# guptakhil/show-tell

Hardware: AMD Instinct MI355X
Metric: training images/sec (ResNet101+GRU, emb=512, bs=128) at 1/2/4/8 MI355X (higher is better)
Workload: dtype bf16; 1 GPU; BASELINE configs[1]: ResNet-101 (train-mode BN, frozen) + 5-layer GRU decoder, E=H=512, V=10000, fwd+bwd+SGD step, synthetic COCO-shaped batch; batch_per_gpu=128, global_batch=128, image=3x224x224, parallelism=dp1

## Files before the change

show-tell_amd/csrc/conv_img.hip:

```cpp
#include "common.h"
#include "prof.h"
#include <stdlib.h>
#include <stdio.h>

namespace {

struct ImgArgs {
  const bf16_t* x; const bf16_t* w; bf16_t* y;
  float* stats; int srep;
  const float* scale; const float* shift; int relu;
  const float* in_stats; const float* in_gamma; const float* in_beta; float in_count, in_eps; int in_srep;
  int B, H, W, N, Wp, R, bands, nbn;
  unsigned long long* stamps;
};

template <int CTRL> __device__ __forceinline__ float dpp_rot_(float v) {
  return __int_as_float(__builtin_amdgcn_update_dpp(0, __float_as_int(v), CTRL, 0xf, 0xf, true));
}
__device__ __forceinline__ float row16_sum_(float v) {
  v += dpp_rot_<0x128>(v); v += dpp_rot_<0x124>(v); v += dpp_rot_<0x122>(v); v += dpp_rot_<0x121>(v);
  return v;
}
__device__ __forceinline__ f32x4 mfma_bf16(const u32x4& a, const u32x4& b, const f32x4& c) {
  return __builtin_amdgcn_mfma_f32_16x16x32_bf16(*reinterpret_cast<const bf16x8*>(&a), *reinterpret_cast<const bf16x8*>(&b), c, 0, 0, 0);
}

template <int NC, int BNLOC>
__device__ __forceinline__ void block_stats_flush(const float (&es)[NC], const float (&ess)[NC], bool writer, int local, char* smem,
                                                  float* sdst, int chan0, int N, int tid) {
  float* sred = reinterpret_cast<float*>(smem);
  __syncthreads();
  if (writer) {
#pragma unroll
    for (int c = 0; c < NC; ++c) { sred[local + c] = es[c]; sred[BNLOC + local + c] = ess[c]; }
  }
  __syncthreads();
  for (int t = tid; t < 2 * BNLOC; t += 256) atomicAdd(sdst + (t < BNLOC ? chan0 + t : N + chan0 + t - BNLOC), sred[t]);
}

__device__ __forceinline__ void bn_relu_chunk(u32x4& v, const float* sc, const float* sh);

template <int C, int TM, int NTW, int HALVES, bool AFFINE, int MS = 1>
__device__ __forceinline__ void conv3x3_img_body(const ImgArgs& a) {
  constexpr int TMW = TM / MS;
  static_assert(TM % MS == 0 && (MS == 1 || MS == 2) && (MS == 1 || HALVES == 1), "position split");
  constexpr int PIX = 2 * C + 32;
  constexpr int CS = C / 32;
  constexpr int CSH = CS / HALVES;
  constexpr int KS = 9 * CS;
  constexpr int CH8 = C / 8;
  constexpr int PSTEP = 256 / CH8;
  constexpr bool ALLW = KS * NTW * 4 <= 96;
  extern __shared__ __attribute__((aligned(16))) char smem[];

  const int tid = threadIdx.x, lane = tid & 63;
  const int wid = __builtin_amdgcn_readfirstlane(tid >> 6);
  int lid;
  {
    const int nblk = gridDim.x, id = blockIdx.x, xcd = id & 7, q = nblk >> 3, r = nblk & 7;
    lid = (xcd < r ? xcd * (q + 1) : r * (q + 1) + (xcd - r) * q) + (id >> 3);
  }
  const int nb = lid % a.nbn;
  const int bi = lid / a.nbn;
  const int band = bi % a.bands, img = bi / a.bands;
  const int r0 = band * a.R;
  const int rows = a.H - r0 < a.R ? a.H - r0 : a.R;
  const int Wp = a.Wp;

#define IMG_STAMP(i) do { if (a.stamps && lane == 0) a.stamps[((size_t)blockIdx.x * 4 + wid) * 8 + (i)] = __builtin_amdgcn_s_memtime(); } while (0)
  IMG_STAMP(0);
  constexpr int NSH = C > 256 ? C / 256 : 1;
  StatHead shd[NSH];
  if (a.in_stats) {
#pragma unroll
    for (int k = 0; k < NSH; ++k) { const int c = (tid + 256 * k) % C; stat_head_issue(shd[k], a.in_stats, a.in_srep, C, c, a.in_gamma, a.in_beta); }
  }
  const int r16 = lane & 15, q4 = lane >> 4;
  const int wn = MS == 1 ? wid : (wid & 1), wm = MS == 1 ? 0 : (wid >> 1);
  const int T0 = (nb * (4 / MS) + wn) * NTW;
  const u32x4* wl = reinterpret_cast<const u32x4*>(a.w) + lane;
  constexpr int WQ = ALLW ? KS : CS;
  u32x4 wq[WQ][NTW];
#pragma unroll
  for (int s = 0; s < WQ; ++s)
#pragma unroll
    for (int j = 0; j < NTW; ++j) wq[s][j] = wl[((size_t)(T0 + j) * KS + s) * 64];

  constexpr int CHH = CH8 / 2, U2 = TM >= 14 ? 19 : TM + 3;
  u32x4 v1[HALVES == 2 ? U2 : 1]; bool ok1[HALVES == 2 ? U2 : 1];
  float sc1[8], sh1[8];
  const int cch2 = tid % CHH, pp2 = tid / CHH;
  const bool xf_ = a.in_stats != nullptr;
  if constexpr (HALVES == 2) {
    const int total = 16 * TM + 2 * Wp + 2;
    float* coef = reinterpret_cast<float*>(smem + (size_t)total * PIX);
    const bf16_t* ximg = a.x + (size_t)img * a.H * a.W * C + cch2 * 8;
    u32x4 v0[U2];
    int pr = pp2 / Wp, pc = pp2 - pr * Wp;
#pragma unroll
    for (int u = 0; u < U2; ++u) {
      const int hi = r0 - 1 + pr, wi = pc - 1;
      ok1[u] = pr < rows + 2 && (unsigned)hi < (unsigned)a.H && (unsigned)wi < (unsigned)a.W;
      const int hc = hi < 0 ? 0 : (hi >= a.H ? a.H - 1 : hi), wc = wi < 0 ? 0 : (wi >= a.W ? a.W - 1 : wi);
      v0[u] = *reinterpret_cast<const u32x4*>(ximg + (size_t)(hc * a.W + wc) * C);
      v1[u] = *reinterpret_cast<const u32x4*>(ximg + (size_t)(hc * a.W + wc) * C + C / 2);
      if (!ok1[u]) { v0[u] = u32x4{0u, 0u, 0u, 0u}; v1[u] = u32x4{0u, 0u, 0u, 0u}; }
      pc += 16;
      while (pc >= Wp) { pc -= Wp; ++pr; }
    }
    float sc0[8], sh0[8];
    if (xf_) {
      const float inv = 1.0f / a.in_count;
#pragma unroll
      for (int k = 0; k < NSH; ++k) {
        const int c = tid + 256 * k;
        if (c < C) stat_head_finish(shd[k], a.in_stats, a.in_srep, C, c, inv, a.in_eps, coef[c], coef[C + c]);
      }
      __syncthreads();
#pragma unroll
      for (int e = 0; e < 8; ++e) {
        sc0[e] = coef[cch2 * 8 + e]; sh0[e] = coef[C + cch2 * 8 + e];
        sc1[e] = coef[C / 2 + cch2 * 8 + e]; sh1[e] = coef[C + C / 2 + cch2 * 8 + e];
      }
    }
#pragma unroll
    for (int u = 0; u < U2; ++u) {
      if (xf_ && ok1[u]) bn_relu_chunk(v0[u], sc0, sh0);
      if (pp2 + 16 * u < total) *reinterpret_cast<u32x4*>(smem + (size_t)(pp2 + 16 * u) * PIX + cch2 * 16) = v0[u];
    }
  } else
  {
    const int cch = tid % CH8;
    float sc[8], sh[8];
    const bool xf = a.in_stats != nullptr;
    const int total = 16 * TM + 2 * Wp + 2;
    float* coef = reinterpret_cast<float*>(smem + (size_t)total * PIX);
    const bf16_t* ximg = a.x + (size_t)img * a.H * a.W * C + cch * 8;
    int pp = tid / CH8;
    int pr = pp / Wp, pc = pp - pr * Wp;
    constexpr int U = C == 256 ? 33 : C == 128 ? 18 : C == 64 ? 12 : 21;
    bool first = true;
    for (; pp < total; pp += U * PSTEP) {
      u32x4 v[U]; bool ok[U]; int dst[U];
#pragma unroll
      for (int u = 0; u < U; ++u) {
        const int hi = r0 - 1 + pr, wi = pc - 1;
        ok[u] = pr < rows + 2 && (unsigned)hi < (unsigned)a.H && (unsigned)wi < (unsigned)a.W;
        dst[u] = pp + u * PSTEP < total ? (pp + u * PSTEP) * PIX + cch * 16 : -1;
        const int hc = hi < 0 ? 0 : (hi >= a.H ? a.H - 1 : hi), wc = wi < 0 ? 0 : (wi >= a.W ? a.W - 1 : wi);
        v[u] = *reinterpret_cast<const u32x4*>(ximg + (size_t)(hc * a.W + wc) * C);
        if (!ok[u]) v[u] = u32x4{0u, 0u, 0u, 0u};
        pc += PSTEP;
        while (pc >= Wp) { pc -= Wp; ++pr; }
      }
      if (xf && first) {
        const float inv = 1.0f / a.in_count;
#pragma unroll
        for (int k = 0; k < NSH; ++k) {
          const int c = tid + 256 * k;
          if (c < C) stat_head_finish(shd[k], a.in_stats, a.in_srep, C, c, inv, a.in_eps, coef[c], coef[C + c]);
        }
        __syncthreads();
#pragma unroll
        for (int e = 0; e < 8; ++e) { sc[e] = coef[cch * 8 + e]; sh[e] = coef[C + cch * 8 + e]; }
        first = false;
      }
#pragma unroll
      for (int u = 0; u < U; ++u) {
        if (xf && ok[u]) {
#pragma unroll
          for (int d = 0; d < 4; ++d) {
            const float lo = fmaxf(__uint_as_float(v[u][d] << 16) * sc[2 * d] + sh[2 * d], 0.f);
            const float hi = fmaxf(__uint_as_float(v[u][d] & 0xffff0000u) * sc[2 * d + 1] + sh[2 * d + 1], 0.f);
            v[u][d] = pack_bf16x2(lo, hi);
          }
        }
        if (dst[u] >= 0) *reinterpret_cast<u32x4*>(smem + dst[u]) = v[u];
      }
    }
  }
  IMG_STAMP(1);
  __syncthreads();
  IMG_STAMP(2);

  f32x4 acc[TMW][NTW];
#pragma unroll
  for (int i = 0; i < TMW; ++i)
#pragma unroll
    for (int j = 0; j < NTW; ++j) acc[i][j] = f32x4{0.f, 0.f, 0.f, 0.f};

  constexpr int TH = TMW > 7 ? 7 : TMW;
  const char* abase = smem + (wm * TMW * 16 + r16) * PIX + q4 * 16;
  auto read_a = [&](u32x4 (&fa)[TMW], int s) {
    const int half = s / (9 * CSH), tap = (s / CSH) % 9, cs = half * CSH + s % CSH;
    const char* ab = abase + ((tap / 3) * Wp + tap % 3) * PIX;
    const char* ab2 = ab + TH * 16 * PIX;
#pragma unroll
    for (int i = 0; i < TMW; ++i)
      fa[i] = i < TH ? *reinterpret_cast<const u32x4*>(ab + i * 16 * PIX + cs * 64) : *reinterpret_cast<const u32x4*>(ab2 + (i - TH) * 16 * PIX + cs * 64);
  };
  u32x4 fa0[TMW], fa1[TMW];
  read_a(fa0, 0);
#pragma clang loop unroll(full)
  for (int s = 0; s < KS; ++s) {
    u32x4 (&cur)[TMW] = (s & 1) ? fa1 : fa0;
    u32x4 (&nxt)[TMW] = (s & 1) ? fa0 : fa1;
    constexpr int SPLIT = HALVES == 2 ? KS / 2 : -1;
    if (s + 1 < KS && s + 1 != SPLIT) read_a(nxt, s + 1);
#pragma unroll
    for (int i = 0; i < TMW; ++i)
#pragma unroll
      for (int j = 0; j < NTW; ++j) acc[i][j] = mfma_bf16(wq[s % WQ][j], cur[i], acc[i][j]);
    if (s + WQ < KS) {
#pragma unroll
      for (int j = 0; j < NTW; ++j) wq[s % WQ][j] = wl[((size_t)(T0 + j) * KS + s + WQ) * 64];
    }
    if constexpr (HALVES == 2) {
      if (s < U2) {
        if (xf_ && ok1[s]) bn_relu_chunk(v1[s], sc1, sh1);
        if (pp2 + 16 * s < 16 * TM + 2 * Wp + 2) *reinterpret_cast<u32x4*>(smem + (size_t)(pp2 + 16 * s) * PIX + C + cch2 * 16) = v1[s];
      }
    }
    __builtin_amdgcn_sched_barrier(0);
    if constexpr (HALVES == 2) {
      if (s + 1 == SPLIT) { __syncthreads(); read_a(nxt, s + 1); }
    }
  }

  IMG_STAMP(3);
  constexpr int NC = 4 * NTW;
  const int cb = T0 * 16 + NC * q4;
  float es[NC], ess[NC], scv[NC], shv[NC];
#pragma unroll
  for (int c = 0; c < NC; ++c) { es[c] = 0.f; ess[c] = 0.f; scv[c] = 1.f; shv[c] = 0.f; }
  if constexpr (AFFINE) {
#pragma unroll
    for (int c = 0; c < NC; ++c) { scv[c] = a.scale[cb + c]; shv[c] = a.shift[cb + c]; }
#pragma unroll
    for (int c = 0; c < NC; ++c) asm volatile("" : "+v"(scv[c]), "+v"(shv[c]));
  }
  int ho = r0, wo = r16 + wm * TMW * 16;
  while (wo >= Wp) { wo -= Wp; ++ho; }
  const long yimg = ((long)img * a.H * a.W * a.N + cb) * 2;
#pragma unroll
  for (int i = 0; i < TMW; ++i) {
    const bool valid = wo < a.W && ho < r0 + rows;
    if (valid) {
      float v[NC];
#pragma unroll
      for (int j = 0; j < NTW; ++j)
#pragma unroll
        for (int e = 0; e < 4; ++e) v[4 * j + e] = acc[i][j][e];
#pragma unroll
      for (int c = 0; c < NC; ++c) { es[c] += v[c]; ess[c] += v[c] * v[c]; }
      if constexpr (AFFINE) {
#pragma unroll
        for (int c = 0; c < NC; ++c) v[c] = v[c] * scv[c] + shv[c];
        if (a.relu) {
#pragma unroll
          for (int c = 0; c < NC; ++c) v[c] = fmaxf(v[c], 0.f);
        }
      }
      const long dst = yimg + (long)(ho * a.W + wo) * a.N * 2;
      if constexpr (NTW == 1) {
        st_out_store8(a.y, dst, u32x2{pack_bf16x2(v[0], v[1]), pack_bf16x2(v[2], v[3])});
      } else {
#pragma unroll
        for (int h = 0; h < NTW / 2; ++h)
          st_out_store16(a.y, dst + 16 * h, u32x4{pack_bf16x2(v[8 * h], v[8 * h + 1]), pack_bf16x2(v[8 * h + 2], v[8 * h + 3]),
                                                  pack_bf16x2(v[8 * h + 4], v[8 * h + 5]), pack_bf16x2(v[8 * h + 6], v[8 * h + 7])});
      }
    }
    wo += 16;
    while (wo >= Wp) { wo -= Wp; ++ho; }
  }
  if (a.stats) {
    float* sdst = a.stats + (a.srep > 1 ? (size_t)(bi % a.srep) * 2 * a.N : 0);
#pragma unroll
    for (int c = 0; c < NC; ++c) { es[c] = row16_sum_(es[c]); ess[c] = row16_sum_(ess[c]); }
    if constexpr (MS == 1) {
      block_stats_flush<NC, 64 * NTW>(es, ess, r16 == 0, wid * 16 * NTW + NC * q4, smem, sdst, nb * 64 * NTW, a.N, tid);
    } else {
      constexpr int BNLOC = (4 / MS) * 16 * NTW;
      float* sred = reinterpret_cast<float*>(smem);
      const int local = wn * 16 * NTW + NC * q4;
      __syncthreads();
      if (r16 == 0 && wm == 0) {
#pragma unroll
        for (int c = 0; c < NC; ++c) { sred[local + c] = es[c]; sred[BNLOC + local + c] = ess[c]; }
      }
      __syncthreads();
      if (r16 == 0 && wm == 1) {
#pragma unroll
        for (int c = 0; c < NC; ++c) { sred[local + c] += es[c]; sred[BNLOC + local + c] += ess[c]; }
      }
      __syncthreads();
      const int chan0 = nb * BNLOC;
      for (int t = tid; t < 2 * BNLOC; t += 256) atomicAdd(sdst + (t < BNLOC ? chan0 + t : a.N + chan0 + t - BNLOC), sred[t]);
    }
  }
  IMG_STAMP(4);
#undef IMG_STAMP
}

template <int C, int TM, int NTW, int HALVES, bool AFFINE>
__global__ __launch_bounds__(256) __attribute__((amdgpu_waves_per_eu(1, 1))) void conv3x3_img_kernel(ImgArgs a) {
  conv3x3_img_body<C, TM, NTW, HALVES, AFFINE>(a);
}
template <int C, int TM, int NTW, int HALVES, bool AFFINE>
__global__ __launch_bounds__(256, 2) void conv3x3_img_kernel_occ2(ImgArgs a) {
  conv3x3_img_body<C, TM, NTW, HALVES, AFFINE, (C == 64 ? 2 : 1)>(a);
}

struct PwArgs {
  const bf16_t* x; const bf16_t* w; bf16_t* y;
  float* stats; int srep;
  const float* scale; const float* shift; int relu;
  const float* in_stats; const float* in_gamma; const float* in_beta; float in_count, in_eps; int in_srep;
  int M, N, nbn, nstage, spb, mbs;
  int Hin, Win, Ho, Wo, stride;
  const bf16_t* res; bf16_t* xout;
  const float* res_stats; const float* res_gamma; const float* res_beta; int res_srep;
  const bf16_t* idn;
};

__device__ __forceinline__ void bn_relu_chunk(u32x4& v, const float* sc, const float* sh) {
#pragma unroll
  for (int d = 0; d < 4; ++d) {
    const float lo = fmaxf(__uint_as_float(v[d] << 16) * sc[2 * d] + sh[2 * d], 0.f);
    const float hi = fmaxf(__uint_as_float(v[d] & 0xffff0000u) * sc[2 * d + 1] + sh[2 * d + 1], 0.f);
    v[d] = pack_bf16x2(lo, hi);
  }
}

template <int K, int NTW, int TMS, int D, bool STRIDED, bool AFFINE, bool FUSE = false, bool RES = false>
__global__ __launch_bounds__(256) void conv1x1_wreg_kernel(PwArgs a) {
  static_assert(!RES || (AFFINE && !STRIDED && !FUSE), "the residual epilogue is the eval-mode conv3 form");
  constexpr int PIX = 2 * K + 32;
  constexpr int KS = K / 32;
  constexpr int CH8 = K / 8;
  constexpr int SM = 16 * TMS;
  constexpr int RPP = 256 / CH8;
  constexpr int NL = SM / RPP;
  static_assert(SM % RPP == 0 && NL >= 1, "stage/loader mismatch");
  constexpr int STAGE_BYTES = SM * PIX;
  extern __shared__ __attribute__((aligned(16))) char smem[];

  const int tid = threadIdx.x, lane = tid & 63;
  const int wid = __builtin_amdgcn_readfirstlane(tid >> 6);
  int lid;
  {
    const int nblk = gridDim.x, id = blockIdx.x, xcd = id & 7, q = nblk >> 3, r = nblk & 7;
    lid = (xcd < r ? xcd * (q + 1) : r * (q + 1) + (xcd - r) * q) + (id >> 3);
  }
  const int slice = lid % a.nbn, mb = lid / a.nbn;
  const int s_begin = 0;
  auto gs = [&](int k) { return a.mbs > 0 ? mb + k * a.mbs : mb * a.spb + k; };
  if (gs(0) >= a.nstage) return;

  const int r16 = lane & 15, q4 = lane >> 4;
  const int T0 = (slice * 4 + wid) * NTW;
  const u32x4* wl = reinterpret_cast<const u32x4*>(a.w) + lane;
  u32x4 wq[KS][NTW];
#pragma unroll
  for (int s = 0; s < KS; ++s)
#pragma unroll
    for (int j = 0; j < NTW; ++j) wq[s][j] = wl[((size_t)(T0 + j) * KS + s) * 64];

  const int cch = tid % CH8, lrow = tid / CH8;
  const bool xf = a.in_stats != nullptr;
  const bool rbn = FUSE && a.res_stats != nullptr;
  float sc[8], sh[8], sc2[FUSE ? 8 : 1], sh2[FUSE ? 8 : 1];
  u32x4 ra[D][NL]; bool rok[D][NL];
  u32x4 rb[FUSE ? D : 1][FUSE ? NL : 1];
  auto gload = [&](u32x4 (&r)[NL], bool (&ok)[NL], int stage, u32x4* q = nullptr) {
#pragma unroll
    for (int i = 0; i < NL; ++i) {
      int m = gs(stage) * SM + lrow + i * RPP;
      ok[i] = m < a.M && stage < a.spb;
      m = ok[i] ? m : a.M - 1;
      long src = m;
      if constexpr (STRIDED) {
        const int hw = a.Ho * a.Wo, b = m / hw, rem = m - b * hw, ho = rem / a.Wo, wo = rem - ho * a.Wo;
        src = ((long)b * a.Hin + ho * a.stride) * a.Win + wo * a.stride;
      }
      r[i] = *reinterpret_cast<const u32x4*>(a.x + src * K + cch * 8);
      if constexpr (FUSE) q[i] = *reinterpret_cast<const u32x4*>(a.res + src * K + cch * 8);
    }
  };
  auto lstore = [&](u32x4 (&r)[NL], bool (&ok)[NL], int buf, int stage = 0, const u32x4* q = nullptr) {
// ... 816 lines not shown
  u32x4 fa0[TM], fa1[TM];
#pragma unroll
  for (int s = 0; s < NSLAB; ++s) {
    const char* ab = abase + (s & 1) * SLAB_BYTES;
    auto read_a = [&](u32x4 (&f)[TM], int kk) {
#pragma unroll
      for (int i = 0; i < TM; ++i) f[i] = *reinterpret_cast<const u32x4*>(ab + i * 16 * PIX + kk * 64);
    };
    read_a(fa0, 0);
#pragma unroll
    for (int kk = 0; kk < KSS; ++kk) {
      const int ks = s * KSS + kk;
      u32x4 (&fa)[TM] = (kk & 1) ? fa1 : fa0;
      u32x4 (&fn)[TM] = (kk & 1) ? fa0 : fa1;
      if (kk + 1 < KSS) read_a(fn, kk + 1);
#pragma unroll
      for (int i = 0; i < TM; ++i)
#pragma unroll
        for (int j = 0; j < NTW; ++j) acc[i][j] = mfma_bf16(wq[ks % WR][j], fa[i], acc[i][j]);
      if (ks + WR < KS) {
#pragma unroll
        for (int j = 0; j < NTW; ++j) wq[ks % WR][j] = wl[((size_t)(T0 + j) * KS + ks + WR) * 64];
      }
      if (s + 1 < NSLAB) {
#pragma unroll
        for (int i = 2 * kk; i < 2 * kk + 2 && i < NL; ++i) { xform1(i, s + 1, (s + 1) & 1); gload1(i, s + 2); }
      }
      __builtin_amdgcn_sched_barrier(0);
    }
    __syncthreads();
  }

  constexpr int NC = 4 * NTW;
  const int cb = T0 * 16 + NC * q4;
  float es[NC], ess[NC];
#pragma unroll
  for (int c = 0; c < NC; ++c) { es[c] = 0.f; ess[c] = 0.f; }
#pragma unroll
  for (int i = 0; i < TM; ++i) {
    const int m = bm * BM + i * 16 + r16;
    if (m < a.M) {
      float v[NC];
#pragma unroll
      for (int j = 0; j < NTW; ++j)
#pragma unroll
        for (int e = 0; e < 4; ++e) v[4 * j + e] = acc[i][j][e];
#pragma unroll
      for (int c = 0; c < NC; ++c) { es[c] += v[c]; ess[c] += v[c] * v[c]; }
      bf16_t* dst = a.y + (size_t)m * N + cb;
#pragma unroll
      for (int h = 0; h < NTW / 2; ++h)
        *reinterpret_cast<u32x4*>(dst + 8 * h) = u32x4{pack_bf16x2(v[8 * h], v[8 * h + 1]), pack_bf16x2(v[8 * h + 2], v[8 * h + 3]),
                                                       pack_bf16x2(v[8 * h + 4], v[8 * h + 5]), pack_bf16x2(v[8 * h + 6], v[8 * h + 7])};
    }
  }
  if (a.stats) {
    float* sdst = a.stats + (a.srep > 1 ? (size_t)(bm % a.srep) * 2 * N : 0);
#pragma unroll
    for (int c = 0; c < NC; ++c) { es[c] = row16_sum_(es[c]); ess[c] = row16_sum_(ess[c]); }
    block_stats_flush<NC, 64 * NTW>(es, ess, r16 == 0, wid * 16 * NTW + NC * q4, smem, sdst, 0, N, tid);
  }
}

#endif

__global__ void pack_frag_kernel(const float* __restrict__ w, bf16_t* __restrict__ out, int Cout, int Cin, int KH, int KW, int ntw, int halves) {
  const long total = (long)Cout * KH * KW * Cin;
  const int KS = KH * KW * Cin / 32;
  const int CH = Cin / halves;
  for (long idx = (long)blockIdx.x * blockDim.x + threadIdx.x; idx < total; idx += (long)gridDim.x * blockDim.x) {
    const int j = idx & 7, lane = (idx >> 3) & 63;
    const long f = idx >> 9;
    const int ks = (int)(f % KS), T = (int)(f / KS);
    const int r16 = lane & 15, q4 = lane >> 4;
    const int ch = (T / ntw) * 16 * ntw + 4 * ntw * (r16 >> 2) + 4 * (T % ntw) + (r16 & 3);
    const int kk = 32 * ks + 8 * q4 + j;
    const int half = kk / (KH * KW * CH), rem = kk - half * KH * KW * CH;
    const int tap = rem / CH, c = half * CH + rem - tap * CH;
    const int kh = tap / KW, kw = tap - kh * KW;
    out[idx] = (bf16_t)w[(((long)ch * Cin + c) * KH + kh) * KW + kw];
  }
}

struct ImgCfg { int tm, ntw; };
inline bool img_cfg(int C, int N, ImgCfg* c) {
  switch (C) {
    case 64:  *c = ImgCfg{16, 2}; return N % 64 == 0;
    case 128: *c = ImgCfg{14, 2}; return N % 128 == 0;
    case 256: *c = ImgCfg{14, 2}; return N % 128 == 0;
    case 512: *c = ImgCfg{4, 2};  return N % 128 == 0;
  }
  return false;
}

template <int C, int TM, int NTW, int HALVES, bool AFFINE>
int launch_img_(const ImgArgs& a, int lds, hipStream_t st, double flops) {
  static int attr_set[64] = {};
  int dev = 0;
  (void)hipGetDevice(&dev);
  constexpr bool OCC2 = C == 64 || (C == 256 && TM == 7);
  if (dev >= 0 && dev < 64 && attr_set[dev] < lds) {
    if constexpr (OCC2) (void)hipFuncSetAttribute(reinterpret_cast<const void*>(&conv3x3_img_kernel_occ2<C, TM, NTW, HALVES, AFFINE>), hipFuncAttributeMaxDynamicSharedMemorySize, 160 * 1024);
    else (void)hipFuncSetAttribute(reinterpret_cast<const void*>(&conv3x3_img_kernel<C, TM, NTW, HALVES, AFFINE>), hipFuncAttributeMaxDynamicSharedMemorySize, 160 * 1024);
    attr_set[dev] = 160 * 1024;
  }
  StProfScope prof(C == 64 ? 8 : C == 128 ? 9 : C == 256 ? 10 : 11, flops, st);
  if constexpr (OCC2) hipLaunchKernelGGL((conv3x3_img_kernel_occ2<C, TM, NTW, HALVES, AFFINE>), dim3(a.B * a.bands * a.nbn), dim3(256), lds, st, a);
  else hipLaunchKernelGGL((conv3x3_img_kernel<C, TM, NTW, HALVES, AFFINE>), dim3(a.B * a.bands * a.nbn), dim3(256), lds, st, a);
  prof.end(st);
  ST_LAUNCH_CHECK();
  return 0;
}

template <int C, int TM, int NTW, int HALVES>
int launch_img(const ImgArgs& a, int lds, hipStream_t st, double flops) {
  return a.scale ? launch_img_<C, TM, NTW, HALVES, true>(a, lds, st, flops) : launch_img_<C, TM, NTW, HALVES, false>(a, lds, st, flops);
}
}

extern "C" int st_conv3x3_img_supported(int H, int W, int C, int N) {
  ImgCfg c;
  if (!img_cfg(C, N, &c)) return 0;
  const int Wp = W + 2;
  if (H < 1 || W < 1 || 16 * c.tm < Wp) return 0;
  const long lds = (long)(16 * c.tm + 2 * Wp + 2) * (2 * C + 32) + 2 * C * (long)sizeof(float);
  return lds <= 160 * 1024 ? (c.ntw | (C == 256 ? 2 << 8 : 0)) : 0;
}

extern "C" int st_conv3x3_img(const st_conv3x3_img_desc* d, void* stream) {
  ST_CHECK(d && d->x && d->w_frag && d->y, "st_conv3x3_img: null pointer");
  ImgCfg c;
  ST_CHECK(st_conv3x3_img_supported(d->H, d->W, d->C, d->N) > 0 && img_cfg(d->C, d->N, &c),
           "st_conv3x3_img: unsupported geometry H=%d W=%d C=%d N=%d", d->H, d->W, d->C, d->N);
  ST_CHECK(d->B > 0 && (long)d->B * d->H * d->W * (d->C > d->N ? d->C : d->N) < (1L << 31), "st_conv3x3_img: bad batch");
  ST_CHECK((d->scale == nullptr) == (d->shift == nullptr) && (d->scale || !d->relu), "st_conv3x3_img: scale, shift (and relu) go together");
  ST_CHECK(!d->in_stats || (d->in_gamma && d->in_beta && d->in_count > 0.f), "st_conv3x3_img: input transform needs gamma, beta, count");
  ST_CHECK(d->stats_replicas >= 0 && d->stats_replicas <= 1024 && d->in_stats_replicas >= 0 && d->in_stats_replicas <= 1024, "st_conv3x3_img: bad stats_replicas");
  ImgArgs a;
  a.x = reinterpret_cast<const bf16_t*>(d->x); a.w = reinterpret_cast<const bf16_t*>(d->w_frag); a.y = reinterpret_cast<bf16_t*>(d->y);
  a.stats = d->stats; a.srep = d->stats_replicas; a.scale = d->scale; a.shift = d->shift; a.relu = d->relu;
  a.in_stats = d->in_stats; a.in_gamma = d->in_gamma; a.in_beta = d->in_beta; a.in_count = d->in_count; a.in_eps = d->in_eps; a.in_srep = d->in_stats_replicas > 1 ? d->in_stats_replicas : 1;
  a.B = d->B; a.H = d->H; a.W = d->W; a.N = d->N; a.Wp = d->W + 2;
  static const bool half_env = [] { const char* e = getenv("ST_IMG256_HALF"); return !e || atoi(e) != 0; }();
  const bool half256 = half_env && d->C == 256 && d->W + 2 <= 16 && d->H > 7 * 16 / (d->W + 2);
  if (half256) c.tm = 7;
  a.R = 16 * c.tm / a.Wp; if (a.R > d->H) a.R = d->H;
  a.bands = (d->H + a.R - 1) / a.R;
  a.nbn = d->C == 64 ? d->N / (32 * c.ntw) : d->N / (64 * c.ntw);
  a.stamps = st_debug_stamps_ptr();
  const int lds = (16 * c.tm + 2 * a.Wp + 2) * (2 * d->C + 32) + 2 * d->C * (int)sizeof(float);
  hipStream_t st = reinterpret_cast<hipStream_t>(stream);
  const double flops = 2.0 * d->B * d->H * d->W * (double)d->N * 9.0 * d->C;
  switch (d->C) {
    case 64:  return launch_img<64, 16, 2, 1>(a, lds, st, flops);
    case 128: return launch_img<128, 14, 2, 1>(a, lds, st, flops);
    case 256: return half256 ? launch_img<256, 7, 2, 2>(a, lds, st, flops) : launch_img<256, 14, 2, 2>(a, lds, st, flops);
    case 512: return launch_img<512, 4, 2, 1>(a, lds, st, flops);
  }
  st_set_error("st_conv3x3_img: no kernel for C=%d", d->C);
  return 1;
}

namespace {
struct PwCfg { int ntw, tms; };
inline bool pw_cfg(int K, int N, PwCfg* c) {
  static const int force = [] { const char* e = getenv("ST_PW_CFG"); int a = 0, b = 0; if (e && sscanf(e, "%d,%d", &a, &b) == 2) return a * 100 + b; return 0; }();
  if (N % 64 || (K != 64 && K != 128 && K != 256 && K != 512)) return false;
  if (force) {
    const int ntw = force / 100, tms = force % 100;
    const bool ok = N % (64 * ntw) == 0 && ((ntw == 1 && (tms == 2 || tms == 4)) || (ntw == 2 && (tms == 2 || tms == 4)) || (ntw == 4 && tms == 4));
    if (ok) { *c = PwCfg{ntw, tms}; return true; }
  }
  const bool n128 = N % 128 == 0;
  switch (K) {
    case 64:  *c = N == 64 ? PwCfg{1, 4} : PwCfg{2, 4}; return N == 64 || n128;
    case 128: *c = n128 ? PwCfg{2, 2} : PwCfg{1, 2}; return true;
    case 256: *c = n128 ? PwCfg{2, 4} : PwCfg{1, 2}; return true;
    case 512: *c = n128 ? PwCfg{2, 2} : PwCfg{1, 2}; return true;
  }
  return false;
}

template <int K, int NTW, int TMS, int D, bool STRIDED, bool AFFINE, bool FUSE = false, bool RES = false>
int launch_pw___(PwArgs& a, hipStream_t st, double flops, bool xf) {
  constexpr int SM = 16 * TMS, PIX = 2 * K + 32;
  const int lds = 2 * SM * PIX + (xf ? (FUSE ? 4 : 2) * K * (int)sizeof(float) : 0);
  a.nbn = a.N / (64 * NTW);
  a.nstage = (a.M + SM - 1) / SM;
  static int attr_set[64] = {};
  static int occ_dev[64] = {};
  int dev = 0;
  (void)hipGetDevice(&dev);
  if (dev < 0 || dev >= 64) dev = 0;
  if (!attr_set[dev] && lds > 64 * 1024) {
    (void)hipFuncSetAttribute(reinterpret_cast<const void*>(&conv1x1_wreg_kernel<K, NTW, TMS, D, STRIDED, AFFINE, FUSE, RES>), hipFuncAttributeMaxDynamicSharedMemorySize, 160 * 1024);
    attr_set[dev] = 1;
  }
  if (!occ_dev[dev]) {
    int nb = 0;
    if (hipOccupancyMaxActiveBlocksPerMultiprocessor(&nb, reinterpret_cast<const void*>(&conv1x1_wreg_kernel<K, NTW, TMS, D, STRIDED, AFFINE, FUSE, RES>), 256, 160 * 1024 / 3) != hipSuccess || nb < 1) nb = 1;
    occ_dev[dev] = nb;
  }
  int occ = (160 * 1024) / lds; if (occ > 3) occ = 3; if (occ > occ_dev[dev]) occ = occ_dev[dev]; if (occ < 1) occ = 1;
  int mbs = (256 * occ) / a.nbn; if (mbs < 1) mbs = 1; if (mbs > a.nstage) mbs = a.nstage;
  a.spb = ((a.nstage + mbs - 1) / mbs + D - 1) / D * D;
  mbs = (a.nstage + a.spb - 1) / a.spb;
  static const bool interleave = [] { const char* e = getenv("ST_PW_INTERLEAVE"); return !e || atoi(e) != 0; }();
  a.mbs = interleave ? mbs : 0;
  StProfScope prof(K == 64 ? 12 : K == 128 ? 13 : K == 256 ? 14 : 15, flops, st);
  hipLaunchKernelGGL((conv1x1_wreg_kernel<K, NTW, TMS, D, STRIDED, AFFINE, FUSE, RES>), dim3(mbs * a.nbn), dim3(256), lds, st, a);
  prof.end(st);
  ST_LAUNCH_CHECK();
  return 0;
}
template <int K, int NTW, int TMS, int D, bool STRIDED>
int launch_pw__(PwArgs& a, hipStream_t st, double flops, bool xf) {
  if constexpr (!STRIDED) { if (a.idn) return launch_pw___<K, NTW, TMS, D, false, true, false, true>(a, st, flops, xf); }
  return a.scale ? launch_pw___<K, NTW, TMS, D, STRIDED, true>(a, st, flops, xf) : launch_pw___<K, NTW, TMS, D, STRIDED, false>(a, st, flops, xf);
}

template <int K, int NTW, int TMS, int D>
int launch_pw_(PwArgs& a, hipStream_t st, double flops, bool xf) {
  return a.stride > 1 ? launch_pw__<K, NTW, TMS, D, true>(a, st, flops, xf) : launch_pw__<K, NTW, TMS, D, false>(a, st, flops, xf);
}

template <int K, int NTW, int TMS>
int launch_pw(PwArgs& a, hipStream_t st, double flops, bool xf) {
  static const int depth = [] { const char* e = getenv("ST_PW_DEPTH"); return e ? atoi(e) : 0; }();
  constexpr int NL = 16 * TMS * K / 2048;
  if constexpr (NL <= 8) { if (depth == 3 || (depth == 0 && NL <= 4)) return launch_pw_<K, NTW, TMS, 3>(a, st, flops, xf); }
  return launch_pw_<K, NTW, TMS, 2>(a, st, flops, xf);
}
}

extern "C" int st_conv1x1_wreg_supported(int K, int N) {
  PwCfg c;
  return pw_cfg(K, N, &c) ? c.ntw : 0;
}

extern "C" int st_conv1x1_wreg(const st_conv1x1_wreg_desc* d, void* stream) {
// ... 254 lines not shown
```

Before: 31930 images/sec.

## Add paired-image conv3x3 form for C=512 and occupancy-2 C=128 form

Adds a band planner header and two new conv3x3 image-kernel forms. For C=512 at 7x7, one block now stacks two images vertically with a shared padding row, so each 16-row MFMA tile wastes fewer positions and the grid is halved. For C=128, a TM=13 form runs two blocks per CU and keeps a single A-fragment buffer, refilling it per tile to cut registers. The cost is extra indexing logic, clamped slot offsets for the padded tail, and different LDS budgets, all behind an environment switch that is on by default.

```diff
diff --git a/show-tell_amd/csrc/conv_img.hip b/show-tell_amd/csrc/conv_img.hip
--- a/show-tell_amd/csrc/conv_img.hip
+++ b/show-tell_amd/csrc/conv_img.hip
@@ -1,5 +1,6 @@
 #include "common.h"
 #include "prof.h"
+#include "img_band.h"
 #include <stdlib.h>
 #include <stdio.h>
 
@@ -40,8 +41,10 @@
 
 __device__ __forceinline__ void bn_relu_chunk(u32x4& v, const float* sc, const float* sh);
 
-template <int C, int TM, int NTW, int HALVES, bool AFFINE, int MS = 1>
+template <int C, int TM, int NTW, int HALVES, bool AFFINE, int MS = 1, int IPW = 1>
 __device__ __forceinline__ void conv3x3_img_body(const ImgArgs& a) {
+  static_assert(IPW == 1 || (IPW == 2 && HALVES == 1 && MS == 1), "image pairs: the plain fill");
+  constexpr bool SA = C == 128 && TM == 13;
   constexpr int TMW = TM / MS;
   static_assert(TM % MS == 0 && (MS == 1 || MS == 2) && (MS == 1 || HALVES == 1), "position split");
   constexpr int PIX = 2 * C + 32;
@@ -64,7 +67,8 @@
   const int bi = lid / a.nbn;
   const int band = bi % a.bands, img = bi / a.bands;
   const int r0 = band * a.R;
-  const int rows = a.H - r0 < a.R ? a.H - r0 : a.R;
+  const int VH = IPW == 1 ? a.H : IPW * (a.H + 1) - 1;
+  const int rows = VH - r0 < a.R ? VH - r0 : a.R;
   const int Wp = a.Wp;
 
 #define IMG_STAMP(i) do { if (a.stamps && lane == 0) a.stamps[((size_t)blockIdx.x * 4 + wid) * 8 + (i)] = __builtin_amdgcn_s_memtime(); } while (0)
@@ -99,9 +103,8 @@
     int pr = pp2 / Wp, pc = pp2 - pr * Wp;
 #pragma unroll
     for (int u = 0; u < U2; ++u) {
-      const int hi = r0 - 1 + pr, wi = pc - 1;
-      ok1[u] = pr < rows + 2 && (unsigned)hi < (unsigned)a.H && (unsigned)wi < (unsigned)a.W;
-      const int hc = hi < 0 ? 0 : (hi >= a.H ? a.H - 1 : hi), wc = wi < 0 ? 0 : (wi >= a.W ? a.W - 1 : wi);
+      int im_, hc, wc;
+      ok1[u] = img_band_pixel_at<1>(a.H, a.W, a.B, img, r0, rows, pr, pc, &im_, &hc, &wc);
       v0[u] = *reinterpret_cast<const u32x4*>(ximg + (size_t)(hc * a.W + wc) * C);
       v1[u] = *reinterpret_cast<const u32x4*>(ximg + (size_t)(hc * a.W + wc) * C + C / 2);
       if (!ok1[u]) { v0[u] = u32x4{0u, 0u, 0u, 0u}; v1[u] = u32x4{0u, 0u, 0u, 0u}; }
@@ -133,22 +136,22 @@
     const int cch = tid % CH8;
     float sc[8], sh[8];
     const bool xf = a.in_stats != nullptr;
-    const int total = 16 * TM + 2 * Wp + 2;
+    const int total = IPW == 1 ? 16 * TM + 2 * Wp + 2 : (VH + 2) * Wp + 2;
     float* coef = reinterpret_cast<float*>(smem + (size_t)total * PIX);
-    const bf16_t* ximg = a.x + (size_t)img * a.H * a.W * C + cch * 8;
+    const bf16_t* ximg = a.x + (IPW == 1 ? (size_t)img * a.H * a.W * C : (size_t)0) + cch * 8;
     int pp = tid / CH8;
     int pr = pp / Wp, pc = pp - pr * Wp;
-    constexpr int U = C == 256 ? 33 : C == 128 ? 18 : C == 64 ? 12 : 21;
+    constexpr int U = C == 256 ? 33 : C == 128 ? 18 : C == 64 ? 12 : IPW == 2 ? 35 : 21;
     bool first = true;
     for (; pp < total; pp += U * PSTEP) {
       u32x4 v[U]; bool ok[U]; int dst[U];
 #pragma unroll
       for (int u = 0; u < U; ++u) {
-        const int hi = r0 - 1 + pr, wi = pc - 1;
-        ok[u] = pr < rows + 2 && (unsigned)hi < (unsigned)a.H && (unsigned)wi < (unsigned)a.W;
+        int im, hc, wc;
+        ok[u] = img_band_pixel_at<IPW>(a.H, a.W, a.B, img, r0, rows, pr, pc, &im, &hc, &wc);
         dst[u] = pp + u * PSTEP < total ? (pp + u * PSTEP) * PIX + cch * 16 : -1;
-        const int hc = hi < 0 ? 0 : (hi >= a.H ? a.H - 1 : hi), wc = wi < 0 ? 0 : (wi >= a.W ? a.W - 1 : wi);
-        v[u] = *reinterpret_cast<const u32x4*>(ximg + (size_t)(hc * a.W + wc) * C);
+        if constexpr (IPW == 1) v[u] = *reinterpret_cast<const u32x4*>(ximg + (size_t)(hc * a.W + wc) * C);
+        else v[u] = *reinterpret_cast<const u32x4*>(ximg + ((size_t)im * a.H * a.W + hc * a.W + wc) * C);
         if (!ok[u]) v[u] = u32x4{0u, 0u, 0u, 0u};
         pc += PSTEP;
         while (pc >= Wp) { pc -= Wp; ++pr; }
@@ -191,26 +194,48 @@
 
   constexpr int TH = TMW > 7 ? 7 : TMW;
   const char* abase = smem + (wm * TMW * 16 + r16) * PIX + q4 * 16;
+  int aoff[IPW == 2 ? TMW : 1];
+  if constexpr (IPW == 2) {
+    const int smax = (VH + 2) * Wp + 2 - 2 * Wp - 3;
+#pragma unroll
+    for (int i = 0; i < TMW; ++i) aoff[i] = (img_band_slot_pixel(i * 16 + r16, smax) - r16) * PIX;
+  }
   auto read_a = [&](u32x4 (&fa)[TMW], int s) {
     const int half = s / (9 * CSH), tap = (s / CSH) % 9, cs = half * CSH + s % CSH;
     const char* ab = abase + ((tap / 3) * Wp + tap % 3) * PIX;
     const char* ab2 = ab + TH * 16 * PIX;
 #pragma unroll
-    for (int i = 0; i < TMW; ++i)
-      fa[i] = i < TH ? *reinterpret_cast<const u32x4*>(ab + i * 16 * PIX + cs * 64) : *reinterpret_cast<const u32x4*>(ab2 + (i - TH) * 16 * PIX + cs * 64);
+    for (int i = 0; i < TMW; ++i) {
+      if constexpr (IPW == 2) fa[i] = *reinterpret_cast<const u32x4*>(ab + aoff[i] + cs * 64);
+      else fa[i] = i < TH ? *reinterpret_cast<const u32x4*>(ab + i * 16 * PIX + cs * 64) : *reinterpret_cast<const u32x4*>(ab2 + (i - TH) * 16 * PIX + cs * 64);
+    }
   };
-  u32x4 fa0[TMW], fa1[TMW];
+  auto read_a1 = [&](u32x4& f, int i, int s) {
+    const int tap = (s / CSH) % 9, cs = s % CSH;
+    const char* ab = abase + ((tap / 3) * Wp + tap % 3) * PIX;
+    f = i < TH ? *reinterpret_cast<const u32x4*>(ab + i * 16 * PIX + cs * 64) : *reinterpret_cast<const u32x4*>(ab + TH * 16 * PIX + (i - TH) * 16 * PIX + cs * 64);
+  };
+  u32x4 fa0[TMW], fa1[SA ? 1 : TMW];
   read_a(fa0, 0);
 #pragma clang loop unroll(full)
   for (int s = 0; s < KS; ++s) {
-    u32x4 (&cur)[TMW] = (s & 1) ? fa1 : fa0;
-    u32x4 (&nxt)[TMW] = (s & 1) ? fa0 : fa1;
+    u32x4 (&cur)[TMW] = (SA || !(s & 1)) ? fa0 : reinterpret_cast<u32x4 (&)[TMW]>(fa1);
+    u32x4 (&nxt)[TMW] = (SA || (s & 1)) ? fa0 : reinterpret_cast<u32x4 (&)[TMW]>(fa1);
     constexpr int SPLIT = HALVES == 2 ? KS / 2 : -1;
+    if constexpr (SA) {
+#pragma unroll
+      for (int i = 0; i < TMW; ++i) {
+#pragma unroll
+        for (int j = 0; j < NTW; ++j) acc[i][j] = mfma_bf16(wq[s % WQ][j], cur[i], acc[i][j]);
+        if (s + 1 < KS) read_a1(cur[i], i, s + 1);
+      }
+    } else {
     if (s + 1 < KS && s + 1 != SPLIT) read_a(nxt, s + 1);
 #pragma unroll
     for (int i = 0; i < TMW; ++i)
 #pragma unroll
       for (int j = 0; j < NTW; ++j) acc[i][j] = mfma_bf16(wq[s % WQ][j], cur[i], acc[i][j]);
+    }
     if (s + WQ < KS) {
 #pragma unroll
       for (int j = 0; j < NTW; ++j) wq[s % WQ][j] = wl[((size_t)(T0 + j) * KS + s + WQ) * 64];
@@ -241,10 +266,11 @@
   }
   int ho = r0, wo = r16 + wm * TMW * 16;
   while (wo >= Wp) { wo -= Wp; ++ho; }
-  const long yimg = ((long)img * a.H * a.W * a.N + cb) * 2;
+  const long yimg = ((long)(IPW == 1 ? img : 0) * a.H * a.W * a.N + cb) * 2;
 #pragma unroll
   for (int i = 0; i < TMW; ++i) {
-    const bool valid = wo < a.W && ho < r0 + rows;
+    int oim, oh;
+    const bool valid = img_band_slot_at<IPW>(a.H, a.W, a.B, img, r0, rows, ho, wo, &oim, &oh);
     if (valid) {
       float v[NC];
 #pragma unroll
@@ -261,7 +287,7 @@
           for (int c = 0; c < NC; ++c) v[c] = fmaxf(v[c], 0.f);
         }
       }
-      const long dst = yimg + (long)(ho * a.W + wo) * a.N * 2;
+      const long dst = yimg + (long)((IPW == 1 ? ho : oim * a.H + oh) * a.W + wo) * a.N * 2;
       if constexpr (NTW == 1) {
         st_out_store8(a.y, dst, u32x2{pack_bf16x2(v[0], v[1]), pack_bf16x2(v[2], v[3])});
       } else {
@@ -303,9 +329,9 @@
 #undef IMG_STAMP
 }
 
-template <int C, int TM, int NTW, int HALVES, bool AFFINE>
+template <int C, int TM, int NTW, int HALVES, bool AFFINE, int IPW = 1>
 __global__ __launch_bounds__(256) __attribute__((amdgpu_waves_per_eu(1, 1))) void conv3x3_img_kernel(ImgArgs a) {
-  conv3x3_img_body<C, TM, NTW, HALVES, AFFINE>(a);
+  conv3x3_img_body<C, TM, NTW, HALVES, AFFINE, 1, IPW>(a);
 }
 template <int C, int TM, int NTW, int HALVES, bool AFFINE>
 __global__ __launch_bounds__(256, 2) void conv3x3_img_kernel_occ2(ImgArgs a) {
@@ -1288,57 +1314,49 @@
   }
 }
 
-struct ImgCfg { int tm, ntw; };
-inline bool img_cfg(int C, int N, ImgCfg* c) {
-  switch (C) {
-    case 64:  *c = ImgCfg{16, 2}; return N % 64 == 0;
-    case 128: *c = ImgCfg{14, 2}; return N % 128 == 0;
-    case 256: *c = ImgCfg{14, 2}; return N % 128 == 0;
-    case 512: *c = ImgCfg{4, 2};  return N % 128 == 0;
-  }
-  return false;
-}
-
-template <int C, int TM, int NTW, int HALVES, bool AFFINE>
+inline bool img_forms_on() { const char* e = getenv("ST_IMG_FORMS"); return !(e && e[0] == '0'); }
+inline bool img_half256_on() { static const bool on = [] { const char* e = getenv("ST_IMG256_HALF"); return !e || atoi(e) != 0; }(); return on; }
+
+template <int C, int TM, int NTW, int HALVES, bool AFFINE, int IPW>
 int launch_img_(const ImgArgs& a, int lds, hipStream_t st, double flops) {
   static int attr_set[64] = {};
   int dev = 0;
   (void)hipGetDevice(&dev);
-  constexpr bool OCC2 = C == 64 || (C == 256 && TM == 7);
+  constexpr bool OCC2 = C == 64 || (C == 256 && TM == 7) || (C == 128 && TM == 13);
+  static_assert(!OCC2 || IPW == 1, "image pairs run one per CU");
   if (dev >= 0 && dev < 64 && attr_set[dev] < lds) {
     if constexpr (OCC2) (void)hipFuncSetAttribute(reinterpret_cast<const void*>(&conv3x3_img_kernel_occ2<C, TM, NTW, HALVES, AFFINE>), hipFuncAttributeMaxDynamicSharedMemorySize, 160 * 1024);
-    else (void)hipFuncSetAttribute(reinterpret_cast<const void*>(&conv3x3_img_kernel<C, TM, NTW, HALVES, AFFINE>), hipFuncAttributeMaxDynamicSharedMemorySize, 160 * 1024);
+    else (void)hipFuncSetAttribute(reinterpret_cast<const void*>(&conv3x3_img_kernel<C, TM, NTW, HALVES, AFFINE, IPW>), hipFuncAttributeMaxDynamicSharedMemorySize, 160 * 1024);
     attr_set[dev] = 160 * 1024;
   }
+  const int grid = ((a.B + IPW - 1) / IPW) * a.bands * a.nbn;
   StProfScope prof(C == 64 ? 8 : C == 128 ? 9 : C == 256 ? 10 : 11, flops, st);
-  if constexpr (OCC2) hipLaunchKernelGGL((conv3x3_img_kernel_occ2<C, TM, NTW, HALVES, AFFINE>), dim3(a.B * a.bands * a.nbn), dim3(256), lds, st, a);
-  else hipLaunchKernelGGL((conv3x3_img_kernel<C, TM, NTW, HALVES, AFFINE>), dim3(a.B * a.bands * a.nbn), dim3(256), lds, st, a);
+  if constexpr (OCC2) hipLaunchKernelGGL((conv3x3_img_kernel_occ2<C, TM, NTW, HALVES, AFFINE>), dim3(grid), dim3(256), lds, st, a);
+  else hipLaunchKernelGGL((conv3x3_img_kernel<C, TM, NTW, HALVES, AFFINE, IPW>), dim3(grid), dim3(256), lds, st, a);
   prof.end(st);
   ST_LAUNCH_CHECK();
   return 0;
 }
 
-template <int C, int TM, int NTW, int HALVES>
+template <int C, int TM, int NTW, int HALVES, int IPW = 1>
 int launch_img(const ImgArgs& a, int lds, hipStream_t st, double flops) {
-  return a.scale ? launch_img_<C, TM, NTW, HALVES, true>(a, lds, st, flops) : launch_img_<C, TM, NTW, HALVES, false>(a, lds, st, flops);
+  return a.scale ? launch_img_<C, TM, NTW, HALVES, true, IPW>(a, lds, st, flops) : launch_img_<C, TM, NTW, HALVES, false, IPW>(a, lds, st, flops);
 }
 }
 
 extern "C" int st_conv3x3_img_supported(int H, int W, int C, int N) {
-  ImgCfg c;
-  if (!img_cfg(C, N, &c)) return 0;
-  const int Wp = W + 2;
-  if (H < 1 || W < 1 || 16 * c.tm < Wp) return 0;
-  const long lds = (long)(16 * c.tm + 2 * Wp + 2) * (2 * C + 32) + 2 * C * (long)sizeof(float);
-  return lds <= 160 * 1024 ? (c.ntw | (C == 256 ? 2 << 8 : 0)) : 0;
+  ImgBand g;
+  if (!img_band_select(&g, H, W, C, N, 1, false, false)) return 0;
+  return g.ntw | (g.halves == 2 ? 2 << 8 : 0);
 }
 
 extern "C" int st_conv3x3_img(const st_conv3x3_img_desc* d, void* stream) {
   ST_CHECK(d && d->x && d->w_frag && d->y, "st_conv3x3_img: null pointer");
-  ImgCfg c;
-  ST_CHECK(st_conv3x3_img_supported(d->H, d->W, d->C, d->N) > 0 && img_cfg(d->C, d->N, &c),
+  ImgBand g;
+  ST_CHECK(st_conv3x3_img_supported(d->H, d->W, d->C, d->N) > 0 && d->B > 0 &&
+           img_band_select(&g, d->H, d->W, d->C, d->N, d->B, img_forms_on(), img_half256_on()),
            "st_conv3x3_img: unsupported geometry H=%d W=%d C=%d N=%d", d->H, d->W, d->C, d->N);
-  ST_CHECK(d->B > 0 && (long)d->B * d->H * d->W * (d->C > d->N ? d->C : d->N) < (1L << 31), "st_conv3x3_img: bad batch");
+  ST_CHECK((long)d->B * d->H * d->W * (d->C > d->N ? d->C : d->N) < (1L << 31), "st_conv3x3_img: bad batch");
   ST_CHECK((d->scale == nullptr) == (d->shift == nullptr) && (d->scale || !d->relu), "st_conv3x3_img: scale, shift (and relu) go together");
   ST_CHECK(!d->in_stats || (d->in_gamma && d->in_beta && d->in_count > 0.f), "st_conv3x3_img: input transform needs gamma, beta, count");
   ST_CHECK(d->stats_replicas >= 0 && d->stats_replicas <= 1024 && d->in_stats_replicas >= 0 && d->in_stats_replicas <= 1024, "st_conv3x3_img: bad stats_replicas");
@@ -1346,22 +1364,21 @@
   a.x = reinterpret_cast<const bf16_t*>(d->x); a.w = reinterpret_cast<const bf16_t*>(d->w_frag); a.y = reinterpret_cast<bf16_t*>(d->y);
   a.stats = d->stats; a.srep = d->stats_replicas; a.scale = d->scale; a.shift = d->shift; a.relu = d->relu;
   a.in_stats = d->in_stats; a.in_gamma = d->in_gamma; a.in_beta = d->in_beta; a.in_count = d->in_count; a.in_eps = d->in_eps; a.in_srep = d->in_stats_replicas > 1 ? d->in_stats_replicas : 1;
-  a.B = d->B; a.H = d->H; a.W = d->W; a.N = d->N; a.Wp = d->W + 2;
-  static const bool half_env = [] { const char* e = getenv("ST_IMG256_HALF"); return !e || atoi(e) != 0; }();
-  const bool half256 = half_env && d->C == 256 && d->W + 2 <= 16 && d->H > 7 * 16 / (d->W + 2);
-  if (half256) c.tm = 7;
-  a.R = 16 * c.tm / a.Wp; if (a.R > d->H) a.R = d->H;
-  a.bands = (d->H + a.R - 1) / a.R;
-  a.nbn = d->C == 64 ? d->N / (32 * c.ntw) : d->N / (64 * c.ntw);
+  a.B = d->B; a.H = d->H; a.W = d->W; a.N = d->N; a.Wp = g.Wp;
+  a.R = g.R; a.bands = g.bands;
+  a.nbn = d->C == 64 ? d->N / (32 * g.ntw) : d->N / (64 * g.ntw);
   a.stamps = st_debug_stamps_ptr();
-  const int lds = (16 * c.tm + 2 * a.Wp + 2) * (2 * d->C + 32) + 2 * d->C * (int)sizeof(float);
+  const int lds = (int)g.lds_bytes;
   hipStream_t st = reinterpret_cast<hipStream_t>(stream);
   const double flops = 2.0 * d->B * d->H * d->W * (double)d->N * 9.0 * d->C;
-  switch (d->C) {
-    case 64:  return launch_img<64, 16, 2, 1>(a, lds, st, flops);
-    case 128: return launch_img<128, 14, 2, 1>(a, lds, st, flops);
-    case 256: return half256 ? launch_img<256, 7, 2, 2>(a, lds, st, flops) : launch_img<256, 14, 2, 2>(a, lds, st, flops);
-    case 512: return launch_img<512, 4, 2, 1>(a, lds, st, flops);
+  switch (g.form) {
+    case IMG_F64:       return launch_img<64, 16, 2, 1>(a, lds, st, flops);
+    case IMG_F128:      return launch_img<128, 14, 2, 1>(a, lds, st, flops);
+    case IMG_F128_OCC2: return launch_img<128, 13, 2, 1>(a, lds, st, flops);
+    case IMG_F256:      return launch_img<256, 14, 2, 2>(a, lds, st, flops);
+    case IMG_F256_HALF: return launch_img<256, 7, 2, 2>(a, lds, st, flops);
+    case IMG_F512:      return launch_img<512, 4, 2, 1>(a, lds, st, flops);
+    case IMG_F512_PAIR: return launch_img<512, 8, 2, 1, 2>(a, lds, st, flops);
   }
   st_set_error("st_conv3x3_img: no kernel for C=%d", d->C);
   return 1;
diff --git a/show-tell_amd/csrc/img_band.h b/show-tell_amd/csrc/img_band.h
--- /dev/null
+++ b/show-tell_amd/csrc/img_band.h
@@ -0,0 +1,112 @@
+#pragma once
+
+#if defined(__HIPCC__)
+#define IMG_BAND_HD __host__ __device__ inline
+#else
+#define IMG_BAND_HD inline
+#endif
+
+enum ImgForm {
+  IMG_F64 = 0,
+  IMG_F128,
+  IMG_F128_OCC2,
+  IMG_F256,
+  IMG_F256_HALF,
+  IMG_F512,
+  IMG_F512_PAIR,
+  IMG_NFORMS
+};
+
+struct ImgBand {
+  int form, C, tm, ntw, halves, occ2, ipw;
+  int H, W, Wp, VH;
+  int R, bands, groups;
+  int slots, tiles;
+  int lds_pixels, smax;
+  long lds_bytes, lds_budget;
+};
+
+IMG_BAND_HD bool img_band_plan(ImgBand* g, int form, int H, int W, int C, int N, int B, bool legacy) {
+  const int fC[IMG_NFORMS]        = {  64,  128,  128,       256,  256,       512,  512 };
+  const int fTm[IMG_NFORMS]       = {  16,  14,   13,        14,   7,         4,    8 };
+  const int fHalves[IMG_NFORMS]   = {  1,   1,    1,         2,    2,         1,    1 };
+  const int fOcc2[IMG_NFORMS]     = {  1,   0,    1,         0,    1,         0,    0 };
+  const int fIpw[IMG_NFORMS]      = {  1,   1,    1,         1,    1,         1,    2 };
+  if (form < 0 || form >= IMG_NFORMS || fC[form] != C || H < 1 || W < 1 || B < 1) return false;
+  if (N <= 0 || N % (C == 64 ? 64 : 128)) return false;
+  if (legacy && (form == IMG_F128_OCC2 || form == IMG_F512_PAIR)) return false;
+  g->form = form; g->C = C; g->tm = fTm[form]; g->ntw = 2; g->halves = fHalves[form]; g->occ2 = fOcc2[form]; g->ipw = fIpw[form];
+  g->H = H; g->W = W; g->Wp = W + (legacy ? 2 : 1);
+  g->VH = g->ipw * (H + 1) - 1;
+  if (16 * g->tm < g->Wp) return false;
+  g->R = 16 * g->tm / g->Wp;
+  if (g->R > g->VH) g->R = g->VH;
+  if (g->ipw > 1 && g->R < g->VH) return false;
+  g->bands = (g->VH + g->R - 1) / g->R;
+  g->groups = (B + g->ipw - 1) / g->ipw;
+  g->slots = g->R * g->Wp;
+  g->tiles = (g->slots + 15) / 16;
+  g->lds_pixels = g->ipw > 1 ? (g->VH + 2) * g->Wp + 2 : 16 * g->tm + 2 * g->Wp + 2;
+  g->smax = g->lds_pixels - 2 * g->Wp - 3;
+  g->lds_bytes = (long)g->lds_pixels * (2 * C + 32) + 2L * C * (long)sizeof(float);
+  g->lds_budget = g->occ2 ? 80 * 1024 : 160 * 1024;
+  return g->lds_bytes <= g->lds_budget;
+}
+
+IMG_BAND_HD bool img_band_select(ImgBand* g, int H, int W, int C, int N, int B, bool forms, bool half256) {
+  ImgBand t;
+  switch (C) {
+    case 64: return img_band_plan(g, IMG_F64, H, W, C, N, B, true);
+    case 128:
+      if (!img_band_plan(g, IMG_F128, H, W, C, N, B, true)) return false;
+      if (forms && img_band_plan(&t, IMG_F128_OCC2, H, W, C, N, B, false) && t.bands == g->bands) *g = t;
+      return true;
+    case 256:
+      if (!img_band_plan(g, IMG_F256, H, W, C, N, B, true)) return false;
+      if (half256 && g->Wp <= 16 && H > 7 * 16 / g->Wp && img_band_plan(&t, IMG_F256_HALF, H, W, C, N, B, true)) *g = t;
+      return true;
+    case 512:
+      if (forms && img_band_plan(&t, IMG_F512_PAIR, H, W, C, N, B, false)) { *g = t; return true; }
+      return img_band_plan(g, IMG_F512, H, W, C, N, B, true);
+  }
+  return false;
+}
+
+template <int IPW>
+IMG_BAND_HD bool img_band_pixel_at(int H, int W, int B, int group, int r0, int rows, int pr, int pc, int* im, int* hc, int* wc) {
+  const int hv = r0 - 1 + pr, wi = pc - 1;
+  int j = 0, hi = hv;
+  if (IPW == 2 && hv > H) { j = 1; hi = hv - H - 1; }
+  int img = group * IPW + j;
+  bool ok = pr < rows + 2 && (unsigned)hi < (unsigned)H && (unsigned)wi < (unsigned)W;
+  if (IPW == 2 && img >= B) { ok = false; img = B - 1; }
+  *im = img;
+  *hc = hi < 0 ? 0 : (hi >= H ? H - 1 : hi);
+  *wc = wi < 0 ? 0 : (wi >= W ? W - 1 : wi);
+  return ok;
+}
+
+template <int IPW>
+IMG_BAND_HD bool img_band_slot_at(int H, int W, int B, int group, int r0, int rows, int hv, int wo, int* im, int* ho) {
+  int j = 0, h = hv;
+  if (IPW == 2 && hv > H) { j = 1; h = hv - H - 1; }
+  *im = group * IPW + j; *ho = h;
+  return wo < W && hv < r0 + rows && (IPW == 1 || (h < H && *im < B));
+}
+
+IMG_BAND_HD int img_band_slot_pixel(int slot, int smax) { return slot < smax ? slot : smax; }
+
+IMG_BAND_HD bool img_band_pixel(const ImgBand& g, int B, int group, int band, int p, int* im, int* h, int* w) {
+  const int r0 = band * g.R, rows = g.VH - r0 < g.R ? g.VH - r0 : g.R, pr = p / g.Wp, pc = p - pr * g.Wp;
+  int hc, wc;
+  const bool ok = g.ipw == 2 ? img_band_pixel_at<2>(g.H, g.W, B, group, r0, rows, pr, pc, im, &hc, &wc)
+                             : img_band_pixel_at<1>(g.H, g.W, B, group, r0, rows, pr, pc, im, &hc, &wc);
+  *h = hc; *w = wc;
+  return ok;
+}
+IMG_BAND_HD bool img_band_slot(const ImgBand& g, int B, int group, int band, int slot, int* im, int* ho, int* wo) {
+  const int r0 = band * g.R, rows = g.VH - r0 < g.R ? g.VH - r0 : g.R, row = slot / g.Wp;
+  *wo = slot - row * g.Wp;
+  return g.ipw == 2 ? img_band_slot_at<2>(g.H, g.W, B, group, r0, rows, r0 + row, *wo, im, ho)
+                    : img_band_slot_at<1>(g.H, g.W, B, group, r0, rows, r0 + row, *wo, im, ho);
+}
```

Result: no change. 32130 images/sec, median of 6 (+0.6%).
